# masapasa/qcpinn-convection-diffusion-qiskit

Hardware: AMD Instinct MI355X
Metric: collocation-points/sec (PDE+BC+IC loss step), 4-qubit cascade (higher is better)
Workload: dtype f32

## Files before the change

### qcpinn-convection-diffusion-qiskit_amd/csrc/qc_mlp.hip

```cpp
#include "qc_internal.h"
#include "qc_philox.h"
#include <tuple>

namespace {

__device__ __forceinline__ float qc_tanh(float x) {
  const float e = __expf(2.f * x);
  return 1.f - 2.f * __builtin_amdgcn_rcpf(e + 1.f);
}

typedef float mf2 __attribute__((ext_vector_type(2)));
__device__ __forceinline__ mf2 m_dup(const float a) { return (mf2){a, a}; }
__device__ __forceinline__ mf2 m_fma(const mf2 a, const mf2 b, const mf2 c) { return __builtin_elementwise_fma(a, b, c); }

__device__ __forceinline__ float analytic_u(float t, float x, float y) {
  const float dx = x - 0.5f, dy = y - 0.5f;
  return expf(-100.f * (dx * dx + dy * dy)) * expf(-t);
}
__device__ __forceinline__ float analytic_r(float t, float x, float y, float D, float vx, float vy) {
  const float u = analytic_u(t, x, y);
  const float dx = x - 0.5f, dy = y - 0.5f;
  const float ut = -u, ux = -200.f * dx * u, uy = -200.f * dy * u;
  const float uxx = (40000.f * dx * dx - 400.f) * u;
  const float uyy = (40000.f * dy * dy - 400.f) * u;
// ... 98 lines not shown
};

template <int N, int K>
__device__ __forceinline__ void pre_blk_load(typename QcPreW<N>::template Blk<K>& w, const float* __restrict__ W1,
                                             const float* __restrict__ b1, const float* __restrict__ W2, const int H,
                                             const int m) {
  const float* __restrict__ p1 = W1 + 3 * m;
  const float* __restrict__ pb = b1 + m;
#pragma unroll
  for (int j = 0; j < 3 * K; ++j) w.w1[j] = p1[j];
#pragma unroll
  for (int j = 0; j < K; ++j) w.b1[j] = pb[j];
#pragma unroll
  for (int i = 0; i < N; ++i) {
    const float* __restrict__ p2 = W2 + (i * H + m);
#pragma unroll
    for (int j = 0; j < K; ++j) w.w2[i][j] = p2[j];
  }
}

template <int N, int NCH, int K>
__device__ __forceinline__ void pre_blk_apply(const typename QcPreW<N>::template Blk<K>& w, const float t, const float x,
                                              const float y, mf2 (&acc2)[NCH == 6 ? 3 : 1][N]) {
  float z[K];
#pragma unroll
  for (int j = 0; j < K; ++j)
    z[j] = qc_tanh(fmaf(w.w1[3 * j], t, fmaf(w.w1[3 * j + 1], x, fmaf(w.w1[3 * j + 2], y, w.b1[j]))));
#pragma unroll
  for (int j = 0; j < K; ++j) {
    if constexpr (NCH == 6) {
      const float w0 = w.w1[3 * j], w1 = w.w1[3 * j + 1], w2 = w.w1[3 * j + 2];
      const float d1 = 1.f - z[j] * z[j], d2 = -2.f * z[j] * d1;
      const mf2 zc2[3] = {(mf2){z[j], d1 * w0}, (mf2){d1 * w1, d1 * w2}, (mf2){d2 * w1 * w1, d2 * w2 * w2}};
#pragma unroll
      for (int i = 0; i < N; ++i) {
        const mf2 wi = m_dup(w.w2[i][j]);
#pragma unroll
        for (int cp = 0; cp < 3; ++cp) acc2[cp][i] = m_fma(wi, zc2[cp], acc2[cp][i]);
      }
    } else {
#pragma unroll
      for (int i = 0; i < N; ++i) acc2[0][i].x = fmaf(w.w2[i][j], z[j], acc2[0][i].x);
    }
  }
}

template <int N, int NCH>
__device__ __forceinline__ void pre_fwd_units(const float* __restrict__ W1, const float* __restrict__ b1,
                                              const float* __restrict__ W2, const int H, const int m0, const int m1,
                                              const float t, const float x, const float y,
                                              mf2 (&acc2)[NCH == 6 ? 3 : 1][N]) {
  constexpr int UB = qc_pre_ub(N);
  qc_unit_blocks<QcPreW<N>, UB, (UB > 1)>(
      m0, m1,
      [&](auto& w, const int m) {
        constexpr int K = std::remove_reference_t<decltype(w)>::count;
        pre_blk_load<N, K>(w, W1, b1, W2, H, m);
      },
      [&](const auto& w, const int) {
        constexpr int K = std::remove_reference_t<decltype(w)>::count;
        pre_blk_apply<N, NCH, K>(w, t, x, y, acc2);
      });
}

template <int N, int NCH, int MAP = 0, bool RF = false>
__device__ __forceinline__ void k_pre_fwd_body(const int64_t bid, const float* __restrict__ X, const float* __restrict__ prm,
                                                 QcLayout L, float* __restrict__ ajets, int64_t B,
                                                 const QcDraw* __restrict__ draw = nullptr, float* __restrict__ Xout = nullptr) {
  __shared__ float s_part[QC_MS][NCH * N][64];
  const int lane = threadIdx.x & 63;
  const int wave = __builtin_amdgcn_readfirstlane(threadIdx.x >> 6);
  const int64_t p = (int64_t)bid * 64 + lane;
  const int64_t pc = p < B ? p : B - 1;
  float t, x, y;
  if (draw != nullptr && draw->enabled) {
    if (NCH == 6) qc_draw_point(0, draw->off_res + pc, 0, draw->seed, draw->step, t, x, y);
    else if (pc < draw->n_ic) qc_draw_point(1, draw->off_ic + pc, 0, draw->seed, draw->step, t, x, y);
    else qc_draw_point<RF>(2, draw->off_bc + (pc - draw->n_ic), draw->face_pts, draw->seed, draw->step, t, x, y);
    if (wave == 0 && p < B) {
      Xout[p * 3 + 0] = t;
      Xout[p * 3 + 1] = x;
      Xout[p * 3 + 2] = y;
    }
  } else {
    t = X[pc * 3 + 0];
    x = X[pc * 3 + 1];
    y = X[pc * 3 + 2];
  }
  constexpr int NP2 = NCH == 6 ? 3 : 1;
  mf2 acc2[NP2][N];
#pragma unroll
  for (int cp = 0; cp < NP2; ++cp)
#pragma unroll
    for (int i = 0; i < N; ++i) acc2[cp][i] = (mf2){0.f, 0.f};
  const float* W1 = prm + L.oW1;
  const float* b1 = prm + L.ob1;
  const float* W2 = prm + L.oW2;
  const int hq = (L.H + QC_MS - 1) / QC_MS;
  const int m0 = wave * hq, m1 = (m0 + hq) < L.H ? (m0 + hq) : L.H;
  pre_fwd_units<N, NCH>(W1, b1, W2, L.H, m0, m1, t, x, y, acc2);
#pragma unroll
  for (int c = 0; c < NCH; ++c)
#pragma unroll
    for (int i = 0; i < N; ++i) s_part[wave][c * N + i][lane] = (c & 1) ? acc2[c >> 1][i].y : acc2[c >> 1][i].x;
  __syncthreads();
  if (p < B) {
    if constexpr (MAP == 0) {
      constexpr int NF = (NCH * N + QC_MS - 1) / QC_MS;
      if constexpr (NF <= 12) {
        float v[NF];
#pragma unroll
        for (int j = 0; j < NF; ++j) {
          const int f = wave + QC_MS * j, fc = f < NCH * N ? f : 0;
          v[j] = (s_part[0][fc][lane] + s_part[1][fc][lane]) + (s_part[2][fc][lane] + s_part[3][fc][lane]);
        }
#pragma unroll
        for (int j = 0; j < NF; ++j) {
          const int f = wave + QC_MS * j;
          if (f < NCH * N) {
            if (f < N) v[j] += prm[L.ob2 + f];
            ajets[(int64_t)f * B + p] = v[j];
          }
        }
      } else {
        for (int f = wave; f < NCH * N; f += QC_MS) {
          float v = (s_part[0][f][lane] + s_part[1][f][lane]) + (s_part[2][f][lane] + s_part[3][f][lane]);
          if (f < N) v += prm[L.ob2 + f];
          ajets[(int64_t)f * B + p] = v;
        }
      }
    } else {
      for (int i = wave; i < N; i += QC_MS) {
        float v[NCH], a[NCH];
#pragma unroll
        for (int c = 0; c < NCH; ++c) {
          const int f = c * N + i;
          v[c] = (s_part[0][f][lane] + s_part[1][f][lane]) + (s_part[2][f][lane] + s_part[3][f][lane]);
        }
        v[0] += prm[L.ob2 + i];
        angle_map_fwd<NCH>(v, a);
#pragma unroll
        for (int c = 0; c < NCH; ++c) ajets[(int64_t)(c * N + i) * B + p] = a[c];
      }
    }
  }
}

template <int N, int NCH, int MAP>
__global__ void __launch_bounds__(256) k_pre_fwd(const float* __restrict__ X, const float* __restrict__ prm,
                                                 QcLayout L, float* __restrict__ ajets, int64_t B) {
  k_pre_fwd_body<N, NCH, MAP>(blockIdx.x, X, prm, L, ajets, B);
}

template <int N, int NCH, int MAP = 0>
__device__ __forceinline__ void k_pre_bwd_body(const int64_t bid, const float* __restrict__ X, const float* __restrict__ prm, QcLayout L,
                          const float* __restrict__ abar, float* __restrict__ part, int64_t part_stride,
                          int64_t row0, int64_t B, int HB, int PS, const float* __restrict__ aj = nullptr) {
  constexpr int NP2 = NCH == 6 ? 3 : 1;
  __shared__ float sX[3][64];
  __shared__ mf2 sA2[NP2 * N][64];
  extern __shared__ float s_acc[];
  const int64_t base = (int64_t)bid * 64;
  const int cnt = (int)((B - base) < 64 ? (B - base) : 64);
  for (int i = threadIdx.x; i < 64 * 3; i += blockDim.x) {
    const int pp = i / 3, k = i % 3;
    sX[k][pp] = pp < cnt ? X[(base + pp) * 3 + k] : 0.f;
  }
  if constexpr (MAP == 0) {
    for (int i = threadIdx.x; i < NCH * N * 64; i += blockDim.x) {
      const int f = i >> 6, pp = i & 63;
      const int c = f / N, w = f % N;
      const float v = pp < cnt ? abar[(int64_t)f * B + base + pp] : 0.f;
      if (c & 1) sA2[(c >> 1) * N + w][pp].y = v;
      else sA2[(c >> 1) * N + w][pp].x = v;
    }
  } else {
    for (int i = threadIdx.x; i < N * 64; i += blockDim.x) {
      const int w = i >> 6, pp = i & 63;
      float ab[NCH], a[NCH], vb[NCH];
#pragma unroll
      for (int c = 0; c < NCH; ++c) {
        const int64_t o = (int64_t)(c * N + w) * B + base + pp;
        ab[c] = pp < cnt ? abar[o] : 0.f;
        a[c] = pp < cnt ? aj[o] : 0.f;
      }
      angle_map_bwd<NCH>(ab, a, vb);
#pragma unroll
      for (int c = 0; c < NCH; ++c) {
        if (c & 1) sA2[(c >> 1) * N + w][pp].y = vb[c];
        else sA2[(c >> 1) * N + w][pp].x = vb[c];
      }
    }
  }
  __syncthreads();

  const int grp = threadIdx.x / HB, m = threadIdx.x % HB;
  const int per = (64 + PS - 1) / PS;
  const int p0 = grp * per, p1 = (p0 + per) < cnt ? (p0 + per) : cnt;
  float gW1[3] = {0.f, 0.f, 0.f}, gb1 = 0.f;
  mf2 gW2p[N];
#pragma unroll
  for (int i = 0; i < N; ++i) gW2p[i] = (mf2){0.f, 0.f};
  if (grp < PS && m < L.H) {
    const float w0 = prm[L.oW1 + 3 * m], w1 = prm[L.oW1 + 3 * m + 1], w2 = prm[L.oW1 + 3 * m + 2];
    const float bb = prm[L.ob1 + m];
    float w2c[N];
#pragma unroll
    for (int i = 0; i < N; ++i) w2c[i] = prm[L.oW2 + i * L.H + m];
    for (int pp = p0; pp < p1; ++pp) {
      const float t = sX[0][pp], x = sX[1][pp], y = sX[2][pp];
      const float h = fmaf(w0, t, fmaf(w1, x, fmaf(w2, y, bb)));
      const float z = qc_tanh(h);
      const float d1 = 1.f - z * z;
      if constexpr (NCH == 6) {
        mf2 a2[3][N], zb2[3];
#pragma unroll
        for (int cp = 0; cp < 3; ++cp) {
          zb2[cp] = (mf2){0.f, 0.f};
#pragma unroll
          for (int i = 0; i < N; ++i) {
            a2[cp][i] = sA2[cp * N + i][pp];
            zb2[cp] = m_fma(m_dup(w2c[i]), a2[cp][i], zb2[cp]);
          }
        }
        const float d2 = -2.f * z * d1;
        const float d3 = -2.f * (d1 * d1 + z * d2);
        const mf2 zc2[3] = {(mf2){z, d1 * w0}, (mf2){d1 * w1, d1 * w2}, (mf2){d2 * w1 * w1, d2 * w2 * w2}};
#pragma unroll
        for (int i = 0; i < N; ++i)
#pragma unroll
          for (int cp = 0; cp < 3; ++cp) gW2p[i] = m_fma(a2[cp][i], zc2[cp], gW2p[i]);
        const float zb[6] = {zb2[0].x, zb2[0].y, zb2[1].x, zb2[1].y, zb2[2].x, zb2[2].y};
        const float hb = zb[0] * d1 + (zb[1] * w0 + zb[2] * w1 + zb[3] * w2) * d2 +
                         (zb[4] * w1 * w1 + zb[5] * w2 * w2) * d3;
        gW1[0] += hb * t + zb[1] * d1;
        gW1[1] += hb * x + zb[2] * d1 + 2.f * zb[4] * d2 * w1;
        gW1[2] += hb * y + zb[3] * d1 + 2.f * zb[5] * d2 * w2;
        gb1 += hb;
      } else {
        float zb0 = 0.f;
#pragma unroll
        for (int i = 0; i < N; ++i) {
          const float a = sA2[i][pp].x;
          zb0 = fmaf(w2c[i], a, zb0);
          gW2p[i].x = fmaf(a, z, gW2p[i].x);
        }
        const float hb = zb0 * d1;
        gW1[0] += hb * t;
        gW1[1] += hb * x;
        gW1[2] += hb * y;
        gb1 += hb;
      }
    }
  }
  if (grp < PS) {
    float* mine = s_acc + (size_t)grp * (4 + N) * HB;
    mine[0 * HB + m] = gW1[0];
    mine[1 * HB + m] = gW1[1];
    mine[2 * HB + m] = gW1[2];
    mine[3 * HB + m] = gb1;
#pragma unroll
    for (int i = 0; i < N; ++i) mine[(4 + i) * HB + m] = gW2p[i].x + gW2p[i].y;
  }
  __syncthreads();
  float* row = part + (row0 + bid) * part_stride;
  if (grp == 0 && m < L.H) {
    float tot[4 + N];
#pragma unroll
    for (int k = 0; k < 4 + N; ++k) {
      float sum = 0.f;
      for (int g2 = 0; g2 < PS; ++g2) sum += s_acc[((size_t)g2 * (4 + N) + k) * HB + m];
      tot[k] = sum;
    }
    row[L.oW1 + 3 * m] = tot[0];
    row[L.oW1 + 3 * m + 1] = tot[1];
    row[L.oW1 + 3 * m + 2] = tot[2];
    row[L.ob1 + m] = tot[3];
#pragma unroll
    for (int i = 0; i < N; ++i) row[L.oW2 + i * L.H + m] = tot[4 + i];
  }
  if (threadIdx.x < N) {
    float sum = 0.f;
    for (int pp = 0; pp < cnt; ++pp) sum += sA2[threadIdx.x][pp].x;
    row[L.ob2 + threadIdx.x] = sum;
  }
}

template <int N, int NCH, int MAP>
__global__ void k_pre_bwd(const float* __restrict__ X, const float* __restrict__ prm, QcLayout L,
                          const float* __restrict__ abar, float* __restrict__ part, int64_t part_stride,
                          int64_t row0, int64_t B, int HB, int PS, const float* __restrict__ aj) {
  k_pre_bwd_body<N, NCH, MAP>(blockIdx.x, X, prm, L, abar, part, part_stride, row0, B, HB, PS, aj);
}

template <int N, int NCH>
__device__ __forceinline__ void post_cotangents(float (&gb)[NCH], float& gw4, const float (&g)[NCH],
                                                const float (&ub)[NCH], const float z, const float w4) {
  const float d1 = 1.f - z * z;
  gw4 = ub[0] * z;
  gb[0] = ub[0] * d1;
  if constexpr (NCH == 6) {
    const float d2 = -2.f * z * d1;
    const float d3 = -2.f * (d1 * d1 + z * d2);
    const float gx2 = g[2] * g[2], gy2 = g[3] * g[3];
    const float lin = ub[1] * g[1] + ub[2] * g[2] + ub[3] * g[3];
    gw4 += d1 * lin + ub[4] * (d2 * gx2 + d1 * g[4]) + ub[5] * (d2 * gy2 + d1 * g[5]);
    gb[0] += d2 * lin + ub[4] * (d3 * gx2 + d2 * g[4]) + ub[5] * (d3 * gy2 + d2 * g[5]);
    gb[1] = ub[1] * d1;
    gb[2] = ub[2] * d1 + 2.f * ub[4] * d2 * g[2];
    gb[3] = ub[3] * d1 + 2.f * ub[5] * d2 * g[3];
    gb[4] = ub[4] * d1;
    gb[5] = ub[5] * d1;
  }
#pragma unroll
  for (int c = 0; c < NCH; ++c) gb[c] *= w4;
}

template <int NCH>
__device__ __forceinline__ void expand_ub(float (&ub)[NCH], float ub0, float gsc, const QcPde& pde) {
  ub[0] = ub0;
  if constexpr (NCH == 6) {
    ub[1] = gsc * pde.c_t;
    ub[2] = gsc * pde.c_x;
    ub[3] = gsc * pde.c_y;
    ub[4] = -pde.d_xx * gsc;
    ub[5] = -pde.d_yy * gsc;
  }
}

__device__ __forceinline__ void learn_coefs(float (&cf)[QC_COEF_N], const float* __restrict__ prm, const QcLayout& L,
                                            const float (&base)[QC_COEF_N], const float (&scale)[QC_COEF_N]) {
  const float* __restrict__ pk = prm + (L.NP - QC_COEF_N);
#pragma unroll
  for (int k = 0; k < QC_COEF_N; ++k) cf[k] = fmaf(scale[k], pk[k], base[k]);
}
__device__ __forceinline__ void learn_columns(float* __restrict__ row, const QcLayout& L, const QcLearn* lr, const int z,
                                              const float (&scale)[QC_COEF_N], const float (&cf)[QC_COEF_N], const float gsc,
                                              const float (&u)[6], const int lane, const bool tile0) {
  float gv[QC_COEF_N] = {gsc * u[0], gsc * u[1], gsc * u[2], gsc * u[3], -gsc * u[4], -gsc * u[5], gsc * (u[0] * u[0] * u[0])};
  qc_wave_sum_multi_to_lane63<QC_COEF_N>(gv);
  if (lane == 63) {
#pragma unroll
    for (int k = 0; k < QC_COEF_N; ++k) row[L.NP - QC_COEF_N + k] = scale[k] == 0.f ? 0.f : scale[k] * gv[k];
    if (tile0) {
      float* hist = (&lr->hist)[z];
      const QcOptState* st = (&lr->st)[z];
      if (hist != nullptr && st != nullptr) {
        const int hi = st->step - st->hist_base;
        if (hi >= 0 && hi < (&lr->hist_cap)[z]) {
#pragma unroll
          for (int k = 0; k < QC_COEF_N; ++k) hist[(int64_t)hi * QC_COEF_N + k] = cf[k];
        }
      }
    }
  }
}
__device__ __forceinline__ int learn_late() {
  int z = 0;
#if defined(__HIP_DEVICE_COMPILE__)
  asm volatile("" : "+s"(z));
#endif
  return z;
}
__device__ __forceinline__ void learn_read(const QcLearn* lr, const int z, float (&base)[QC_COEF_N], float (&scale)[QC_COEF_N]) {
#pragma unroll
  for (int k = 0; k < QC_COEF_N; ++k) {
    base[k] = lr->base[k + z];
    scale[k] = lr->scale[k + z];
  }
}
__device__ __forceinline__ void learn_zero_columns(float* __restrict__ row, const QcLayout& L) {
#pragma unroll
  for (int k = 0; k < QC_COEF_N; ++k) row[L.NP - QC_COEF_N + k] = 0.f;
}

template <int NCH>
__device__ __forceinline__ void bal_weights(QcPde& pde, const float* __restrict__ prm, const QcLayout& L, const QcBal* bl) {
  const float* __restrict__ pk = prm + (L.NP - QC_BAL_N);
  auto uniform = [](const float v) {
    return __builtin_bit_cast(float, __builtin_amdgcn_readfirstlane(__builtin_bit_cast(int, v)));
  };
  if constexpr (NCH == 6) {
    pde.w_res = uniform(pde.w_res * qc_bal_factor(bl->scale[0], pk[0]));
  } else {
    pde.w_val_b = uniform(pde.w_val_b * qc_bal_factor(bl->scale[1], pk[1]));
    pde.w_val_a = uniform(pde.w_val_a * qc_bal_factor(bl->scale[2], pk[2]));
  }
}
__device__ __forceinline__ void bal_zero_columns(float* __restrict__ row, const QcLayout& L) {
#pragma unroll
  for (int k = 0; k < QC_BAL_N; ++k) row[L.NP - QC_BAL_N + k] = 0.f;
}

template <int N, int NCH, int MODE, bool DATA = false, bool COEF = false, bool LEARN = false, bool BAL = false>
__device__ __forceinline__ void k_post_body(const int64_t bid, const float* __restrict__ X, const float* __restrict__ prm, QcLayout L,
                                              QcPde pde, const float* __restrict__ qjets,
                                              float* __restrict__ out_u, float* __restrict__ out_res,
                                              const float* __restrict__ in_ubar, const float* __restrict__ in_rbar,
                                              float* __restrict__ qbar, float* __restrict__ part,
                                              int64_t part_stride, int64_t row0, int64_t B,
                                              const float* __restrict__ tg = nullptr, const float c_u = 0.f,
                                              const float* __restrict__ coef = nullptr, const QcLearn* lr = nullptr,
                                              const QcBal* bl = nullptr) {
  static_assert(!DATA || MODE == 2, "tabulated targets: the fused mode only");
  static_assert(!COEF || (DATA && NCH == 6), "per-point operators: tabulated residual points only");
  static_assert(!LEARN || (DATA && !COEF), "learned operators: tabulated targets, no table");
  static_assert(!BAL || (DATA && !COEF && !LEARN), "balanced weights: the tabulated kind's operator");
  constexpr bool OPC = COEF || (LEARN && NCH == 6);
  __shared__ float s_buf[QC_MS][NCH * N][64];
  const int lane = threadIdx.x & 63;
  const int wave = __builtin_amdgcn_readfirstlane(threadIdx.x >> 6);
  const int64_t tile = bid;
  const int64_t p = tile * 64 + lane;
  const bool live = p < B;
  const int64_t pc = live ? p : B - 1;
  float q[NCH][N];
#pragma unroll
  for (int c = 0; c < NCH; ++c)
#pragma unroll
    for (int i = 0; i < N; ++i) q[c][i] = qjets[((int64_t)c * N + i) * B + pc];
  float cf[OPC ? QC_COEF_N : 1];
  if constexpr (COEF) {
#pragma unroll
    for (int k = 0; k < QC_COEF_N; ++k) cf[k] = coef[(int64_t)k * B + pc];
  }
// ... 120 lines not shown
            row[L.NP + 0] = ls;
            row[L.NP + 1] = 0.f;
            row[L.NP + 2] = 0.f;
            if constexpr (BAL) bal_zero_columns(row, L);
          }
          if constexpr (LEARN) learn_columns(row, L, lr, 0, lscale, cf, gsc, u, lane, tile == 0);
        }
      } else {
        const bool seg_a = p < pde.n_seg_a;
        const float target = DATA ? tgp : value_target(pde, seg_a, t, x, y);
        const float e = live ? u[0] - target : 0.f;
        ub0 = (seg_a ? pde.w_val_a : pde.w_val_b) * e;
        if (wave == 0) {
          const float la = qc_wave_sum_to_lane63(seg_a ? e * e * pde.inv_n_a : 0.f);
          const float lb = qc_wave_sum_to_lane63(seg_a ? 0.f : e * e * pde.inv_n_b);
          if (lane == 63) {
            row[L.NP + 0] = 0.f;
            row[L.NP + 1] = lb;
            row[L.NP + 2] = la;
            if constexpr (LEARN) learn_zero_columns(row, L);
            if constexpr (BAL) bal_zero_columns(row, L);
          }
        }
      }
      if constexpr (OPC) {
        if (live && wave == 0) {
          out_u[p] = ub0;
          out_u[B + p] = gsc * cf[1];
          out_u[2 * B + p] = gsc * cf[2];
          out_u[3 * B + p] = gsc * cf[3];
          out_u[4 * B + p] = -cf[4] * gsc;
          out_u[5 * B + p] = -cf[5] * gsc;
        }
      } else if (live && wave == 0) {
        out_u[p] = ub0;
        if constexpr (NCH == 6) out_res[p] = gsc;
      }
    }
  }
  if constexpr (MODE == 1) {
    ub0 = (live && in_ubar) ? in_ubar[pc] : 0.f;
    if constexpr (NCH == 6) gsc = (live && in_rbar) ? in_rbar[pc] : 0.f;
  }
  if constexpr (MODE == 2) {
    const float scale = NCH == 6 ? gsc : ub0;
#pragma unroll
    for (int c = 0; c < NCH; ++c)
#pragma unroll
      for (int i = 0; i < N; ++i) {
        if constexpr (OPC) s_buf[wave][c * N + i][lane] = scale * (c == 0 ? fmaf(k3, qbu0[i], qbu[c][i]) : qbu[c][i]);
        else s_buf[wave][c * N + i][lane] = scale * qbu[c][i];
      }
    __syncthreads();
    if (live) {
      for (int f = wave; f < NCH * N; f += QC_MS)
        qbar[(int64_t)f * B + p] = (s_buf[0][f][lane] + s_buf[1][f][lane]) + (s_buf[2][f][lane] + s_buf[3][f][lane]);
    }
  }
  if constexpr (MODE == 1 || MODE == 3) {
    float ub[NCH];
    if constexpr (MODE == 3) {
#pragma unroll
      for (int c = 0; c < NCH; ++c) ub[c] = live ? in_ubar[(int64_t)c * B + pc] : 0.f;
    } else {
      expand_ub<NCH>(ub, ub0, gsc, pde);
    }
    float qb[NCH][N];
#pragma unroll
    for (int c = 0; c < NCH; ++c)
#pragma unroll
      for (int i = 0; i < N; ++i) qb[c][i] = 0.f;
    for (int m = m0; m < m1; ++m) {
      float g[NCH];
#pragma unroll
      for (int c = 0; c < NCH; ++c) {
        float sum = (c == 0) ? b3[m] : 0.f;
#pragma unroll
        for (int i = 0; i < N; ++i) sum = fmaf(W3[m * N + i], q[c][i], sum);
        g[c] = sum;
      }
      const float z = qc_tanh(g[0]);
      float gb[NCH], gw4;
      post_cotangents<N, NCH>(gb, gw4, g, ub, z, W4[m]);
#pragma unroll
      for (int i = 0; i < N; ++i) {
        const float w3 = W3[m * N + i];
#pragma unroll
        for (int c = 0; c < NCH; ++c) qb[c][i] = fmaf(w3, gb[c], qb[c][i]);
      }
    }
#pragma unroll
    for (int c = 0; c < NCH; ++c)
#pragma unroll
      for (int i = 0; i < N; ++i) s_buf[wave][c * N + i][lane] = qb[c][i];
    __syncthreads();
    if (live) {
      for (int f = wave; f < NCH * N; f += QC_MS)
        qbar[(int64_t)f * B + p] = (s_buf[0][f][lane] + s_buf[1][f][lane]) + (s_buf[2][f][lane] + s_buf[3][f][lane]);
    }
  }
}

template <class... TG>
struct QcKind {
  static_assert(sizeof...(TG) <= 2, "(), (QcTab), (QcTab, const float*), (QcTab, QcLearn) or (QcTab, QcBal)");
  static constexpr bool data = sizeof...(TG) >= 1;
  static constexpr bool learn = (std::is_same_v<TG, QcLearn> || ...);
  static constexpr bool bal = (std::is_same_v<TG, QcBal> || ...);
  static constexpr bool coef = sizeof...(TG) == 2 && !learn && !bal;
  static __device__ __forceinline__ const float* tg_res(const TG&... t) {
    if constexpr (data) return std::get<0>(std::tie(t...)).tg_res; else return nullptr;
  }
  static __device__ __forceinline__ const float* tg_val(const TG&... t) {
    if constexpr (data) return std::get<0>(std::tie(t...)).tg_val; else return nullptr;
  }
  static __device__ __forceinline__ float c_u(const TG&... t) {
    if constexpr (data && !coef && !learn) return std::get<0>(std::tie(t...)).c_u; else return 0.f;
  }
  static __device__ __forceinline__ const QcLearn* op(const TG&... t) {
    if constexpr (learn) return &std::get<1>(std::tie(t...)); else return nullptr;
  }
  static __device__ __forceinline__ const QcBal* weights(const TG&... t) {
    if constexpr (bal) return &std::get<1>(std::tie(t...)); else return nullptr;
  }
  static __device__ __forceinline__ const float* table(const TG&... t) {
    if constexpr (coef) return std::get<1>(std::tie(t...)); else return nullptr;
  }
};

template <int N, int NCH, int MODE, class... TG>
__global__ void __launch_bounds__(256) k_post(const float* __restrict__ X, const float* __restrict__ prm, QcLayout L,
                                              QcPde pde, const float* __restrict__ qjets,
                                              float* __restrict__ out_u, float* __restrict__ out_res,
                                              const float* __restrict__ in_ubar, const float* __restrict__ in_rbar,
                                              float* __restrict__ qbar, float* __restrict__ part,
                                              int64_t part_stride, int64_t row0, int64_t B, TG... tg) {
  using K = QcKind<TG...>;
  k_post_body<N, NCH, MODE, K::data, K::coef, K::learn, K::bal>(blockIdx.x, X, prm, L, pde, qjets, out_u, out_res, in_ubar, in_rbar,
                                                                qbar, part, part_stride, row0, B,
                                                                NCH == 6 ? K::tg_res(tg...) : K::tg_val(tg...), K::c_u(tg...),
                                                                K::table(tg...), K::op(tg...), K::weights(tg...));
}

template <int N, int NCH>
__device__ __forceinline__ void k_post_wg_body(const int64_t bid, const float* __restrict__ prm, QcLayout L, QcPde pde, const float* __restrict__ qjets,
                          const float* __restrict__ ubar, const float* __restrict__ rbar,
                          float* __restrict__ part, int64_t part_stride, int64_t row0, int64_t B, int HB, int PS,
                          int gen = 0) {
  __shared__ float sQ[NCH * N][64];
  __shared__ float sU[NCH == 6 ? 6 : 2][64];
  extern __shared__ float s_acc[];
  const int64_t base = (int64_t)bid * 64;
  const int cnt = (int)((B - base) < 64 ? (B - base) : 64);
  for (int i = threadIdx.x; i < NCH * N * 64; i += blockDim.x) {
    const int f = i >> 6, pp = i & 63;
    sQ[f][pp] = pp < cnt ? qjets[(int64_t)f * B + base + pp] : 0.f;
  }
  if (NCH == 6 && gen) {
    for (int i = threadIdx.x; i < 6 * 64; i += blockDim.x) {
      const int k = i >> 6, pp = i & 63;
      sU[k][pp] = pp < cnt ? ubar[(int64_t)k * B + base + pp] : 0.f;
    }
  } else {
    for (int i = threadIdx.x; i < 128; i += blockDim.x) {
      const int k = i >> 6, pp = i & 63;
      const float* src = k == 0 ? ubar : rbar;
      sU[k][pp] = (pp < cnt && src != nullptr) ? src[base + pp] : 0.f;
    }
  }
  __syncthreads();
  const int grp = threadIdx.x / HB, m = threadIdx.x % HB;
  const int per = (64 + PS - 1) / PS;
  const int p0 = grp * per, p1 = (p0 + per) < cnt ? (p0 + per) : cnt;
  float gW3[N], gb3 = 0.f, gW4 = 0.f;
#pragma unroll
  for (int i = 0; i < N; ++i) gW3[i] = 0.f;
  if (grp < PS && m < L.H) {
    float w3[N];
#pragma unroll
    for (int i = 0; i < N; ++i) w3[i] = prm[L.oW3 + m * N + i];
    const float b3m = prm[L.ob3 + m], w4 = prm[L.oW4 + m];
    for (int pp = p0; pp < p1; ++pp) {
      float g[NCH];
#pragma unroll
      for (int c = 0; c < NCH; ++c) {
        float sum = (c == 0) ? b3m : 0.f;
#pragma unroll
        for (int i = 0; i < N; ++i) sum = fmaf(w3[i], sQ[c * N + i][pp], sum);
        g[c] = sum;
      }
      const float z = qc_tanh(g[0]);
      float ub[NCH];
      if (NCH == 6 && gen) {
#pragma unroll
        for (int c = 0; c < NCH; ++c) ub[c] = sU[c < (NCH == 6 ? 6 : 2) ? c : 0][pp];
      } else {
        expand_ub<NCH>(ub, sU[0][pp], sU[1][pp], pde);
      }
      float gb[NCH], gw4;
      post_cotangents<N, NCH>(gb, gw4, g, ub, z, w4);
      gW4 += gw4;
      gb3 += gb[0];
#pragma unroll
      for (int i = 0; i < N; ++i) {
        float sum = gW3[i];
#pragma unroll
        for (int c = 0; c < NCH; ++c) sum = fmaf(gb[c], sQ[c * N + i][pp], sum);
        gW3[i] = sum;
      }
    }
  }
  if (grp < PS) {
    float* mine = s_acc + (size_t)grp * (N + 2) * HB;
#pragma unroll
    for (int i = 0; i < N; ++i) mine[i * HB + m] = gW3[i];
    mine[N * HB + m] = gb3;
    mine[(N + 1) * HB + m] = gW4;
  }
  __syncthreads();
  float* row = part + (row0 + bid) * part_stride;
  if (grp == 0 && m < L.H) {
    float tot[N + 2];
#pragma unroll
    for (int k = 0; k < N + 2; ++k) {
      float sum = 0.f;
      for (int g2 = 0; g2 < PS; ++g2) sum += s_acc[((size_t)g2 * (N + 2) + k) * HB + m];
      tot[k] = sum;
    }
#pragma unroll
    for (int i = 0; i < N; ++i) row[L.oW3 + m * N + i] = tot[i];
    row[L.ob3 + m] = tot[N];
    row[L.oW4 + m] = tot[N + 1];
  }
  if (threadIdx.x == 0) {
    float sum = 0.f;
    for (int pp = 0; pp < cnt; ++pp) sum += sU[0][pp];
    row[L.ob4] = sum;
  }
}

template <int N, int NCH>
__global__ void k_post_wg(const float* __restrict__ prm, QcLayout L, QcPde pde, const float* __restrict__ qjets,
                          const float* __restrict__ ubar, const float* __restrict__ rbar,
                          float* __restrict__ part, int64_t part_stride, int64_t row0, int64_t B, int HB, int PS, int gen) {
  k_post_wg_body<N, NCH>(blockIdx.x, prm, L, pde, qjets, ubar, rbar, part, part_stride, row0, B, HB, PS, gen);
}

template <int N, int MAP = 0, bool RF = false>
__device__ __forceinline__ void k_pre_fwd_value4(const int64_t bid, const float* __restrict__ X, const float* __restrict__ prm,
                                                 QcLayout L, float* __restrict__ ajets, int64_t B,
                                                 const QcDraw* __restrict__ draw, float* __restrict__ Xout) {
  const int lane = threadIdx.x & 63;
  const int wave = __builtin_amdgcn_readfirstlane(threadIdx.x >> 6);
  const int64_t tile = bid * 4 + wave;
  if (tile * 64 >= B) return;
  const int64_t p = tile * 64 + lane;
  const int64_t pc = p < B ? p : B - 1;
  float t, x, y;
  if (draw != nullptr && draw->enabled) {
    if (pc < draw->n_ic) qc_draw_point(1, draw->off_ic + pc, 0, draw->seed, draw->step, t, x, y);
    else qc_draw_point<RF>(2, draw->off_bc + (pc - draw->n_ic), draw->face_pts, draw->seed, draw->step, t, x, y);
    if (p < B) {
      Xout[p * 3 + 0] = t;
      Xout[p * 3 + 1] = x;
      Xout[p * 3 + 2] = y;
    }
  } else {
    t = X[pc * 3 + 0];
    x = X[pc * 3 + 1];
    y = X[pc * 3 + 2];
  }
  const float* W1 = prm + L.oW1;
  const float* b1 = prm + L.ob1;
  const float* W2 = prm + L.oW2;
  const int hq = (L.H + QC_MS - 1) / QC_MS;
  float part[QC_MS][N];
#pragma unroll
  for (int k = 0; k < QC_MS; ++k) {
    mf2 acc[1][N];
#pragma unroll
    for (int i = 0; i < N; ++i) acc[0][i] = (mf2){0.f, 0.f};
    const int m0 = k * hq, m1 = (m0 + hq) < L.H ? (m0 + hq) : L.H;
    pre_fwd_units<N, 1>(W1, b1, W2, L.H, m0, m1, t, x, y, acc);
#pragma unroll
    for (int i = 0; i < N; ++i) part[k][i] = acc[0][i].x;
  }
  if (p < B) {
#pragma unroll
    for (int i = 0; i < N; ++i) {
      const float v = ((part[0][i] + part[1][i]) + (part[2][i] + part[3][i])) + prm[L.ob2 + i];
      if constexpr (MAP == 0) {
        ajets[(int64_t)i * B + p] = v;
      } else {
        const float vv[1] = {v};
        float a[1];
        angle_map_fwd<1>(vv, a);
        ajets[(int64_t)i * B + p] = a[0];
      }
    }
  }
}

template <int N, bool DATA = false, bool LEARN = false, bool BAL = false>
__device__ __forceinline__ void k_post_value4(const int64_t bid, const float* __restrict__ X, const float* __restrict__ prm,
                                              QcLayout L, QcPde pde, const float* __restrict__ qjets,
                                              float* __restrict__ out_u, float* __restrict__ qbar, float* __restrict__ part,
                                              int64_t part_stride, int64_t row0, int64_t B,
                                              const float* __restrict__ tg = nullptr, const QcBal* bl = nullptr) {
  const int lane = threadIdx.x & 63;
  const int wave = __builtin_amdgcn_readfirstlane(threadIdx.x >> 6);
  const int64_t tile = bid * 4 + wave;
  if (tile * 64 >= B) return;
  const int64_t p = tile * 64 + lane;
  const bool live = p < B;
  const int64_t pc = live ? p : B - 1;
  float q[N];
#pragma unroll
  for (int i = 0; i < N; ++i) q[i] = qjets[(int64_t)i * B + pc];
  const float* W3 = prm + L.oW3;
  const float* b3 = prm + L.ob3;
  const float* W4 = prm + L.oW4;
  const int hq = (L.H + QC_MS - 1) / QC_MS;
  float up[QC_MS], qbu[QC_MS][N];
#pragma unroll
  for (int k = 0; k < QC_MS; ++k) {
    up[k] = 0.f;
#pragma unroll
    for (int i = 0; i < N; ++i) qbu[k][i] = 0.f;
    const int m0 = k * hq, m1 = (m0 + hq) < L.H ? (m0 + hq) : L.H;
    for (int m = m0; m < m1; ++m) {
      float g = b3[m];
#pragma unroll
      for (int i = 0; i < N; ++i) g = fmaf(W3[m * N + i], q[i], g);
      const float z = qc_tanh(g);
      const float w4 = W4[m];
      up[k] = fmaf(w4, z, up[k]);
      const float gb = (1.f - z * z) * w4;
#pragma unroll
      for (int i = 0; i < N; ++i) qbu[k][i] = fmaf(W3[m * N + i], gb, qbu[k][i]);
    }
  }
  const float u = ((up[0] + up[1]) + (up[2] + up[3])) + prm[L.ob4];
  const bool seg_a = p < pde.n_seg_a;
  float target;
  if constexpr (DATA) {
    target = tg[pc];
  } else {
    const float t = X[pc * 3 + 0], x = X[pc * 3 + 1], y = X[pc * 3 + 2];
    target = value_target(pde, seg_a, t, x, y);
  }
  if constexpr (BAL) bal_weights<1>(pde, prm, L, bl);
  const float e = live ? u - target : 0.f;
  const float ub0 = (seg_a ? pde.w_val_a : pde.w_val_b) * e;
  const float la = qc_wave_sum_to_lane63(seg_a ? e * e * pde.inv_n_a : 0.f);
  const float lb = qc_wave_sum_to_lane63(seg_a ? 0.f : e * e * pde.inv_n_b);
  if (lane == 63) {
    float* row = part + (row0 + tile) * part_stride;
    row[L.NP + 0] = 0.f;
    row[L.NP + 1] = lb;
    row[L.NP + 2] = la;
    if constexpr (LEARN) learn_zero_columns(row, L);
    if constexpr (BAL) bal_zero_columns(row, L);
  }
  if (live) {
    out_u[p] = ub0;
#pragma unroll
    for (int i = 0; i < N; ++i)
      qbar[(int64_t)i * B + p] = (ub0 * qbu[0][i] + ub0 * qbu[1][i]) + (ub0 * qbu[2][i] + ub0 * qbu[3][i]);
  }
}

constexpr int QC_POST_VALUE_TPB = 1;

template <int N>
struct QcPostW {
  template <int K>
  struct Blk { static constexpr int count = K; float w3[K][N], b3[K], w4[K]; };
};
template <int N, int K>
__device__ __forceinline__ void post_blk_load(typename QcPostW<N>::template Blk<K>& w, const float* __restrict__ W3,
// ... 1187 lines not shown
```

Before: 603.5 million.

## Batch global-to-shared staging loads per wave in pre/post backward kernels

For small qubit counts, the backward pre-MLP and post-MLP weight-gradient kernels now stage abar, aj, qjets and ubar rows through registers. Each wave issues several row loads at once using a scalar-base address and clamped lane offsets. Parameter loads are hoisted ahead of the shared-memory stores, and empty asm pins keep the compiler from serializing the loads. The cross-group reduction of partial sums now reads several groups at a time. The aim is more memory-level parallelism and less load latency in the staging phase, at the cost of more registers and more complex code.

```diff
diff --git a/qcpinn-convection-diffusion-qiskit_amd/csrc/qc_mlp.hip b/qcpinn-convection-diffusion-qiskit_amd/csrc/qc_mlp.hip
--- a/qcpinn-convection-diffusion-qiskit_amd/csrc/qc_mlp.hip
+++ b/qcpinn-convection-diffusion-qiskit_amd/csrc/qc_mlp.hip
@@ -274,6 +274,56 @@
   k_pre_fwd_body<N, NCH, MAP>(blockIdx.x, X, prm, L, ajets, B);
 }
 
+__device__ __forceinline__ float qc_row_load(const float* __restrict__ row, const unsigned lane_off) {
+#if defined(__HIP_DEVICE_COMPILE__)
+  using G = const __attribute__((address_space(1))) char*;
+  G b = (G)row;
+  asm("" : "+s"(b));
+  return *(const __attribute__((address_space(1))) float*)(b + (size_t)(lane_off * 4u));
+#else
+  return row[lane_off];
+#endif
+}
+__device__ __forceinline__ void qc_pin(float& v) {
+#if defined(__HIP_DEVICE_COMPILE__)
+  asm volatile("" : "+v"(v));
+#endif
+}
+template <int A, int B2>
+__device__ __forceinline__ void qc_pin(float (&v)[A][B2]) {
+#pragma unroll
+  for (int a = 0; a < A; ++a)
+#pragma unroll
+    for (int b = 0; b < B2; ++b) qc_pin(v[a][b]);
+}
+template <int A>
+__device__ __forceinline__ void qc_pin(float (&v)[A]) {
+#pragma unroll
+  for (int a = 0; a < A; ++a) qc_pin(v[a]);
+}
+
+template <int K>
+__device__ __forceinline__ void qc_group_sums(const float* s_acc, const int PS, const int HB, const int m, float (&tot)[K]) {
+  constexpr int GC = K >= 40 ? 1 : 40 / K;
+#pragma unroll
+  for (int k = 0; k < K; ++k) tot[k] = 0.f;
+  for (int g0 = 0; g0 < PS; g0 += GC) {
+    float v[GC][K];
+#pragma unroll
+    for (int j = 0; j < GC; ++j) {
+      const int gc = (g0 + j) < PS ? (g0 + j) : PS - 1;
+#pragma unroll
+      for (int k = 0; k < K; ++k) v[j][k] = s_acc[((size_t)gc * K + k) * HB + m];
+    }
+#pragma unroll
+    for (int j = 0; j < GC; ++j)
+#pragma unroll
+      for (int k = 0; k < K; ++k) tot[k] += (g0 + j) < PS ? v[j][k] : 0.f;
+  }
+}
+
+constexpr bool qc_stage_batched(const int n) { return n <= 8; }
+
 template <int N, int NCH, int MAP = 0>
 __device__ __forceinline__ void k_pre_bwd_body(const int64_t bid, const float* __restrict__ X, const float* __restrict__ prm, QcLayout L,
                           const float* __restrict__ abar, float* __restrict__ part, int64_t part_stride,
@@ -284,39 +334,124 @@
   extern __shared__ float s_acc[];
   const int64_t base = (int64_t)bid * 64;
   const int cnt = (int)((B - base) < 64 ? (B - base) : 64);
-  for (int i = threadIdx.x; i < 64 * 3; i += blockDim.x) {
-    const int pp = i / 3, k = i % 3;
-    sX[k][pp] = pp < cnt ? X[(base + pp) * 3 + k] : 0.f;
-  }
-  if constexpr (MAP == 0) {
-    for (int i = threadIdx.x; i < NCH * N * 64; i += blockDim.x) {
-      const int f = i >> 6, pp = i & 63;
-      const int c = f / N, w = f % N;
-      const float v = pp < cnt ? abar[(int64_t)f * B + base + pp] : 0.f;
-      if (c & 1) sA2[(c >> 1) * N + w][pp].y = v;
-      else sA2[(c >> 1) * N + w][pp].x = v;
+  int grp, m;
+  float w0, w1, w2, bb, w2c[N];
+  constexpr bool BATCH = qc_stage_batched(N);
+  if constexpr (BATCH) {
+    const int lane = threadIdx.x & 63;
+    const int wave = __builtin_amdgcn_readfirstlane(threadIdx.x >> 6), nw = blockDim.x >> 6;
+    const bool live = lane < cnt;
+    const unsigned pc = live ? lane : cnt - 1;
+    constexpr int NR = MAP == 0 ? NP2 * N : N;
+    constexpr int NV = MAP == 0 ? (NCH == 6 ? 2 : 1) : 2 * NCH;
+    constexpr int CH = NV == 12 ? 1 : 8 / NV;
+    auto request = [&](const int r0, float (&v)[CH][NV]) {
+#pragma unroll
+      for (int j = 0; j < CH; ++j) {
+        const int r = r0 + j * nw, rc = r < NR ? r : 0;
+        if constexpr (MAP == 0) {
+          const int cp = rc / N, w = rc % N;
+#pragma unroll
+          for (int q = 0; q < NV; ++q) v[j][q] = qc_row_load(abar + ((int64_t)((2 * cp + q) * N + w) * B + base), pc);
+        } else {
+#pragma unroll
+          for (int c = 0; c < NCH; ++c) {
+            const int64_t o = (int64_t)(c * N + rc) * B + base;
+            v[j][c] = qc_row_load(abar + o, pc);
+            v[j][NCH + c] = qc_row_load(aj + o, pc);
+          }
+        }
+      }
+    };
+    auto put = [&](const int r0, const float (&v)[CH][NV]) {
+#pragma unroll
+      for (int j = 0; j < CH; ++j) {
+        const int r = r0 + j * nw;
+        if (r < NR) {
+          if constexpr (MAP == 0) {
+            if constexpr (NCH == 6) sA2[r][lane] = (mf2){live ? v[j][0] : 0.f, live ? v[j][1] : 0.f};
+            else sA2[r][lane].x = live ? v[j][0] : 0.f;
+          } else {
+            float ab[NCH], a[NCH], vb[NCH];
+#pragma unroll
+            for (int c = 0; c < NCH; ++c) {
+              ab[c] = live ? v[j][c] : 0.f;
+              a[c] = live ? v[j][NCH + c] : 0.f;
+            }
+            angle_map_bwd<NCH>(ab, a, vb);
+            if constexpr (NCH == 6) {
+#pragma unroll
+              for (int cp = 0; cp < 3; ++cp) sA2[cp * N + r][lane] = (mf2){vb[2 * cp], vb[2 * cp + 1]};
+            } else {
+              sA2[r][lane].x = vb[0];
+            }
+          }
+        }
+      }
+    };
+    float stg[CH][NV];
+    request(wave, stg);
+    const int xi = (wave < 3 ? wave : 0) * 64 + lane;
+    float xv = qc_row_load(X + base * 3, xi < 3 * cnt ? xi : 3 * cnt - 1);
+    grp = threadIdx.x / HB, m = threadIdx.x % HB;
+    const int mc = m < L.H ? m : L.H - 1;
+    w0 = prm[L.oW1 + 3 * mc], w1 = prm[L.oW1 + 3 * mc + 1], w2 = prm[L.oW1 + 3 * mc + 2];
+    bb = prm[L.ob1 + mc];
+#pragma unroll
+    for (int i = 0; i < N; ++i) w2c[i] = prm[L.oW2 + i * L.H + mc];
+    qc_pin(stg);
+    qc_pin(xv);
+    qc_pin(w0);
+    qc_pin(w1);
+    qc_pin(w2);
+    qc_pin(bb);
+    qc_pin(w2c);
+    if (wave < 3) sX[xi % 3][xi / 3] = xi < 3 * cnt ? xv : 0.f;
+    put(wave, stg);
+    for (int r = wave + nw; r < 3; r += nw) {
+      const int i = r * 64 + lane;
+      sX[i % 3][i / 3] = i < 3 * cnt ? X[base * 3 + i] : 0.f;
+    }
+    for (int r0 = wave + CH * nw; r0 < NR; r0 += CH * nw) {
+      request(r0, stg);
+      qc_pin(stg);
+      put(r0, stg);
     }
   } else {
-    for (int i = threadIdx.x; i < N * 64; i += blockDim.x) {
-      const int w = i >> 6, pp = i & 63;
-      float ab[NCH], a[NCH], vb[NCH];
-#pragma unroll
-      for (int c = 0; c < NCH; ++c) {
-        const int64_t o = (int64_t)(c * N + w) * B + base + pp;
-        ab[c] = pp < cnt ? abar[o] : 0.f;
-        a[c] = pp < cnt ? aj[o] : 0.f;
-      }
-      angle_map_bwd<NCH>(ab, a, vb);
-#pragma unroll
-      for (int c = 0; c < NCH; ++c) {
-        if (c & 1) sA2[(c >> 1) * N + w][pp].y = vb[c];
-        else sA2[(c >> 1) * N + w][pp].x = vb[c];
+    for (int i = threadIdx.x; i < 64 * 3; i += blockDim.x) {
+      const int pp = i / 3, k = i % 3;
+      sX[k][pp] = pp < cnt ? X[(base + pp) * 3 + k] : 0.f;
+    }
+    if constexpr (MAP == 0) {
+      for (int i = threadIdx.x; i < NCH * N * 64; i += blockDim.x) {
+        const int f = i >> 6, pp = i & 63;
+        const int c = f / N, w = f % N;
+        const float v = pp < cnt ? abar[(int64_t)f * B + base + pp] : 0.f;
+        if (c & 1) sA2[(c >> 1) * N + w][pp].y = v;
+        else sA2[(c >> 1) * N + w][pp].x = v;
+      }
+    } else {
+      for (int i = threadIdx.x; i < N * 64; i += blockDim.x) {
+        const int w = i >> 6, pp = i & 63;
+        float ab[NCH], a[NCH], vb[NCH];
+#pragma unroll
+        for (int c = 0; c < NCH; ++c) {
+          const int64_t o = (int64_t)(c * N + w) * B + base + pp;
+          ab[c] = pp < cnt ? abar[o] : 0.f;
+          a[c] = pp < cnt ? aj[o] : 0.f;
+        }
+        angle_map_bwd<NCH>(ab, a, vb);
+#pragma unroll
+        for (int c = 0; c < NCH; ++c) {
+          if (c & 1) sA2[(c >> 1) * N + w][pp].y = vb[c];
+          else sA2[(c >> 1) * N + w][pp].x = vb[c];
+        }
       }
     }
   }
   __syncthreads();
 
-  const int grp = threadIdx.x / HB, m = threadIdx.x % HB;
+  if constexpr (!BATCH) grp = threadIdx.x / HB, m = threadIdx.x % HB;
   const int per = (64 + PS - 1) / PS;
   const int p0 = grp * per, p1 = (p0 + per) < cnt ? (p0 + per) : cnt;
   float gW1[3] = {0.f, 0.f, 0.f}, gb1 = 0.f;
@@ -324,11 +459,12 @@
 #pragma unroll
   for (int i = 0; i < N; ++i) gW2p[i] = (mf2){0.f, 0.f};
   if (grp < PS && m < L.H) {
-    const float w0 = prm[L.oW1 + 3 * m], w1 = prm[L.oW1 + 3 * m + 1], w2 = prm[L.oW1 + 3 * m + 2];
-    const float bb = prm[L.ob1 + m];
-    float w2c[N];
-#pragma unroll
-    for (int i = 0; i < N; ++i) w2c[i] = prm[L.oW2 + i * L.H + m];
+    if constexpr (!BATCH) {
+      w0 = prm[L.oW1 + 3 * m], w1 = prm[L.oW1 + 3 * m + 1], w2 = prm[L.oW1 + 3 * m + 2];
+      bb = prm[L.ob1 + m];
+#pragma unroll
+      for (int i = 0; i < N; ++i) w2c[i] = prm[L.oW2 + i * L.H + m];
+    }
     for (int pp = p0; pp < p1; ++pp) {
       const float t = sX[0][pp], x = sX[1][pp], y = sX[2][pp];
       const float h = fmaf(w0, t, fmaf(w1, x, fmaf(w2, y, bb)));
@@ -388,11 +524,15 @@
   float* row = part + (row0 + bid) * part_stride;
   if (grp == 0 && m < L.H) {
     float tot[4 + N];
-#pragma unroll
-    for (int k = 0; k < 4 + N; ++k) {
-      float sum = 0.f;
-      for (int g2 = 0; g2 < PS; ++g2) sum += s_acc[((size_t)g2 * (4 + N) + k) * HB + m];
-      tot[k] = sum;
+    if constexpr (BATCH) {
+      qc_group_sums<4 + N>(s_acc, PS, HB, m, tot);
+    } else {
+#pragma unroll
+      for (int k = 0; k < 4 + N; ++k) {
+        float sum = 0.f;
+        for (int g2 = 0; g2 < PS; ++g2) sum += s_acc[((size_t)g2 * (4 + N) + k) * HB + m];
+        tot[k] = sum;
+      }
     }
     row[L.oW1 + 3 * m] = tot[0];
     row[L.oW1 + 3 * m + 1] = tot[1];
@@ -819,34 +959,115 @@
   extern __shared__ float s_acc[];
   const int64_t base = (int64_t)bid * 64;
   const int cnt = (int)((B - base) < 64 ? (B - base) : 64);
-  for (int i = threadIdx.x; i < NCH * N * 64; i += blockDim.x) {
-    const int f = i >> 6, pp = i & 63;
-    sQ[f][pp] = pp < cnt ? qjets[(int64_t)f * B + base + pp] : 0.f;
-  }
-  if (NCH == 6 && gen) {
-    for (int i = threadIdx.x; i < 6 * 64; i += blockDim.x) {
-      const int k = i >> 6, pp = i & 63;
-      sU[k][pp] = pp < cnt ? ubar[(int64_t)k * B + base + pp] : 0.f;
+  int grp, m;
+  float w3[N], b3m, w4;
+  constexpr bool BATCH = qc_stage_batched(N);
+  if constexpr (BATCH) {
+    const int lane = threadIdx.x & 63;
+    const int wave = __builtin_amdgcn_readfirstlane(threadIdx.x >> 6), nw = blockDim.x >> 6;
+    const bool live = lane < cnt;
+    const unsigned pc = live ? lane : cnt - 1;
+    constexpr int NRQ = NCH * N, CHQ = 8, CHU = 2;
+    const int NRU = (NCH == 6 && gen) ? 6 : 2;
+    auto request_q = [&](const int r0, float (&v)[CHQ]) {
+#pragma unroll
+      for (int j = 0; j < CHQ; ++j) {
+        const int r = r0 + j * nw, rc = r < NRQ ? r : 0;
+        v[j] = qc_row_load(qjets + ((int64_t)rc * B + base), pc);
+      }
+    };
+    auto put_q = [&](const int r0, const float (&v)[CHQ]) {
+#pragma unroll
+      for (int j = 0; j < CHQ; ++j) {
+        const int r = r0 + j * nw;
+        if (r < NRQ) sQ[r][lane] = live ? v[j] : 0.f;
+      }
+    };
+    auto source_u = [&](const int r) -> const float* {
+      if (r >= NRU) return nullptr;
+      if (NCH == 6 && gen) return ubar + ((int64_t)r * B + base);
+      const float* src = r == 0 ? ubar : rbar;
+      return src != nullptr ? src + base : nullptr;
+    };
+    auto request_u = [&](const int r0, float (&v)[CHU]) {
+#pragma unroll
+      for (int j = 0; j < CHU; ++j) {
+        const float* src = source_u(r0 + j * nw);
+        v[j] = qc_row_load(src != nullptr ? src : qjets + base, pc);
+      }
+    };
+    auto put_u = [&](const int r0, const float (&v)[CHU]) {
+#pragma unroll
+      for (int j = 0; j < CHU; ++j) {
+        const int r = r0 + j * nw;
+        if (r < NRU) sU[r][lane] = (live && source_u(r) != nullptr) ? v[j] : 0.f;
+      }
+    };
+    const bool batch_u = NCH == 1 || gen;
+    float stq[CHQ], stu[CHU];
+    request_q(wave, stq);
+    if (batch_u) request_u(wave, stu);
+    grp = threadIdx.x / HB, m = threadIdx.x % HB;
+    const int mc = m < L.H ? m : L.H - 1;
+#pragma unroll
+    for (int i = 0; i < N; ++i) w3[i] = prm[L.oW3 + mc * N + i];
+    b3m = prm[L.ob3 + mc], w4 = prm[L.oW4 + mc];
+    qc_pin(stq);
+    if (batch_u) qc_pin(stu);
+    qc_pin(w3);
+    qc_pin(b3m);
+    qc_pin(w4);
+    put_q(wave, stq);
+    if (batch_u) put_u(wave, stu);
+    for (int r0 = wave + CHQ * nw; r0 < NRQ; r0 += CHQ * nw) {
+      request_q(r0, stq);
+      qc_pin(stq);
+      put_q(r0, stq);
+    }
+    if (batch_u) {
+      for (int r0 = wave + CHU * nw; r0 < NRU; r0 += CHU * nw) {
+        request_u(r0, stu);
+        qc_pin(stu);
+        put_u(r0, stu);
+      }
+    } else {
+      for (int i = threadIdx.x; i < 128; i += blockDim.x) {
+        const int k = i >> 6, pp = i & 63;
+        const float* src = k == 0 ? ubar : rbar;
+        sU[k][pp] = (pp < cnt && src != nullptr) ? src[base + pp] : 0.f;
+      }
     }
   } else {
-    for (int i = threadIdx.x; i < 128; i += blockDim.x) {
-      const int k = i >> 6, pp = i & 63;
-      const float* src = k == 0 ? ubar : rbar;
-      sU[k][pp] = (pp < cnt && src != nullptr) ? src[base + pp] : 0.f;
+    for (int i = threadIdx.x; i < NCH * N * 64; i += blockDim.x) {
+      const int f = i >> 6, pp = i & 63;
+      sQ[f][pp] = pp < cnt ? qjets[(int64_t)f * B + base + pp] : 0.f;
+    }
+    if (NCH == 6 && gen) {
+      for (int i = threadIdx.x; i < 6 * 64; i += blockDim.x) {
+        const int k = i >> 6, pp = i & 63;
+        sU[k][pp] = pp < cnt ? ubar[(int64_t)k * B + base + pp] : 0.f;
+      }
+    } else {
+      for (int i = threadIdx.x; i < 128; i += blockDim.x) {
+        const int k = i >> 6, pp = i & 63;
+        const float* src = k == 0 ? ubar : rbar;
+        sU[k][pp] = (pp < cnt && src != nullptr) ? src[base + pp] : 0.f;
+      }
     }
   }
   __syncthreads();
-  const int grp = threadIdx.x / HB, m = threadIdx.x % HB;
+  if constexpr (!BATCH) grp = threadIdx.x / HB, m = threadIdx.x % HB;
   const int per = (64 + PS - 1) / PS;
   const int p0 = grp * per, p1 = (p0 + per) < cnt ? (p0 + per) : cnt;
   float gW3[N], gb3 = 0.f, gW4 = 0.f;
 #pragma unroll
   for (int i = 0; i < N; ++i) gW3[i] = 0.f;
   if (grp < PS && m < L.H) {
-    float w3[N];
-#pragma unroll
-    for (int i = 0; i < N; ++i) w3[i] = prm[L.oW3 + m * N + i];
-    const float b3m = prm[L.ob3 + m], w4 = prm[L.oW4 + m];
+    if constexpr (!BATCH) {
+#pragma unroll
+      for (int i = 0; i < N; ++i) w3[i] = prm[L.oW3 + m * N + i];
+      b3m = prm[L.ob3 + m], w4 = prm[L.oW4 + m];
+    }
     for (int pp = p0; pp < p1; ++pp) {
       float g[NCH];
 #pragma unroll
@@ -888,11 +1109,15 @@
   float* row = part + (row0 + bid) * part_stride;
   if (grp == 0 && m < L.H) {
     float tot[N + 2];
-#pragma unroll
-    for (int k = 0; k < N + 2; ++k) {
-      float sum = 0.f;
-      for (int g2 = 0; g2 < PS; ++g2) sum += s_acc[((size_t)g2 * (N + 2) + k) * HB + m];
-      tot[k] = sum;
+    if constexpr (BATCH) {
+      qc_group_sums<N + 2>(s_acc, PS, HB, m, tot);
+    } else {
+#pragma unroll
+      for (int k = 0; k < N + 2; ++k) {
+        float sum = 0.f;
+        for (int g2 = 0; g2 < PS; ++g2) sum += s_acc[((size_t)g2 * (N + 2) + k) * HB + m];
+        tot[k] = sum;
+      }
     }
 #pragma unroll
     for (int i = 0; i < N; ++i) row[L.oW3 + m * N + i] = tot[i];
```

Measured after the change: 609.6 million, median of 6. 1.0% higher.
